# pinellolab/CRISPR-HAWK

Measured on AMD Instinct MI355X. Metric: candidate guides scored/sec, higher is better.
Workload: dtype u32

## Files before the change

### crispr-hawk_amd/csrc/hawk_api_cldict.hip

```cpp
#include <hip/hip_runtime.h>

#include <algorithm>
#include <cstdio>
#include <cstdlib>

#include "hawk_host.h"

static_assert(CL_MAX_ROWS == HAWK_ROW_MAX_HAP, "cl_build_sizes declines the rows the packed layout cannot hold");

enum ClBuildEvent { EV_BUILD_BEGIN = 8, EV_BUILD_END = 9 };

struct ClZero {
  char* base;
  const ClBuildSizes* z;
  template <class T> T* at(size_t off) const { return reinterpret_cast<T*>(base + off); }
  uint32_t* status() const { return at<uint32_t>(z->z_status); }
  uint32_t* counters() const { return at<uint32_t>(z->z_counters); }
  ClResults* results() const { return at<ClResults>(z->z_results); }
  uint32_t* cnt() const { return at<uint32_t>(z->z_cnt); }
  uint32_t* lcnt() const { return at<uint32_t>(z->z_lcnt); }
  uint32_t* claim() const { return at<uint32_t>(z->z_claim); }
  unsigned long long* vdesc() const { return at<unsigned long long>(z->z_vdesc); }
  uint32_t* span2() const { return at<uint32_t>(z->z_span2); }
  ClSlot* tab() const { return at<ClSlot>(z->z_tab); }
};

static int dict_reserve(hawk_xplan* x, const ClBuildSizes& sz, PoolScope& tmp, ClZero* zero, ClBuild* b) {
  ClusterDictionary& cl = x->cl;
  const uint32_t n = x->n_hap;
  zero->z = &sz;
  TEMPCHK(tmp, &zero->base, sz.z_end);
  ClChunks& ch = b->ch;
  TEMPCHK(tmp, &ch.ch_off, (size_t)(n + 1) * 4);
  TEMPCHK(tmp, &ch.ch_row, (size_t)sz.ch_bound * 4);
  TEMPCHK(tmp, &ch.inst_base, (size_t)(sz.ch_bound + 1) * 4);
  TEMPCHK(tmp, &ch.list_base, (size_t)(sz.ch_bound + 1) * 4);
  TEMPCHK(tmp, &b->list.list, (size_t)sz.inst_bound * sizeof(ClListed));
  TEMPCHK(tmp, &b->list.state, (size_t)sz.inst_bound * 4);
  for (DevBuf* buf : {&cl.inst_uid, &cl.inst_o, &cl.inst_row, &cl.inst_pa, &cl.inst_rb})
    if (int rc = buf->reserve((size_t)sz.inst_bound * 4)) return rc;
  ch.ch_bound = sz.ch_bound; ch.cnt = zero->cnt(); ch.lcnt = zero->lcnt();
  b->list.bound = sz.inst_bound;
  ClPlan& p = b->plan;
  p.heads = x->heads.p; p.hv_off = x->off.as<uint64_t>(); p.hap_len = x->hlen.as<uint32_t>();
  p.ss = x->m_ss.as<int32_t>(); p.se = x->m_se.as<int32_t>(); p.is_ref = x->m_is_ref.as<uint8_t>();
  p.seg_off = x->m_seg_off.as<uint32_t>(); p.seg_rel = x->m_seg_rel.as<uint32_t>();
  p.n_rows = n; p.n_var = x->n_var;
  b->var.desc = zero->vdesc(); b->var.claim = zero->claim();
  ClInst& ci = b->inst;
  ci.o = cl.inst_o.as<int32_t>(); ci.row = cl.inst_row.as<uint32_t>(); ci.pa = cl.inst_pa.as<int32_t>(); ci.rb = cl.inst_rb.as<int32_t>();
  ci.uid = cl.inst_uid.as<uint32_t>();
  b->tally.counters = zero->counters(); b->tally.results = zero->results(); b->tally.status = zero->status();
  return HAWK_OK;
}

static void dict_cut(hipStream_t st, const ClBuild& b) {
  const ClChunks& ch = b.ch;
  hawk_launch_cl_chunks(st, b);
  hawk_launch_cl_count(st, b);
  if (hawk_cl_head_chunks(ch.ch_bound))
    hawk_launch_scan2_u32(st, ch.cnt, ch.lcnt, ch.ch_bound, ch.inst_base, ch.list_base, b.var.desc, b.var.claim, b.plan.n_var);
  else
    hawk_launch_scan2_u32(st, ch.cnt, ch.lcnt, ch.ch_bound, ch.inst_base, ch.list_base);
}

static int dict_attempt(hawk_xplan* x, const ClBuild& b, const ClTable& t, uint32_t* span2, ClResults* res) {
  ClusterDictionary& cl = x->cl;
  hawk_ctx* ctx = x->ctx;
  hipStream_t st = ctx->stream;
  for (DevBuf* buf : {&cl.u_rec, &cl.u_n, &cl.u_row, &cl.u_o, &cl.u_seg})
    if (int rc = buf->reserve((size_t)t.u_cap * 4)) return rc;
  ClUniq cu;
  cu.rec = cl.u_rec.as<uint32_t>(); cu.n = cl.u_n.as<uint32_t>(); cu.row = cl.u_row.as<uint32_t>(); cu.o = cl.u_o.as<int32_t>();
  cu.seg = cl.u_seg.as<uint32_t>(); cu.span2 = span2;
  hawk_launch_cl_fill(st, b);
// ... 23 lines not shown
int xplan_build_dict(hawk_xplan* x) {
  ClusterDictionary& cl = x->cl;
  if (cl.built) return HAWK_OK;
  cl.built = true; cl.usable = false; cl.status = 0; cl.n_inst = cl.n_uniq = cl.n_real = 0; cl.slots = 0; cl.build_ms = 0.f;
  hawk_ctx* ctx = x->ctx;
  hipStream_t st = ctx->stream;
  const ClBuildSizes sz = cl_build_sizes(x->ncar, x->n_hap, x->n_var, cl.last_uniq);
  if (sz.declined) { cl.status = CL_ST_DECLINED; return HAWK_OK; }
  PoolScope tmp;
  ClZero zero;
  ClBuild b = {};
  int rc;
  if ((rc = dict_reserve(x, sz, tmp, &zero, &b))) return rc;
  HIPCHK(hipEventRecord(ctx->ev[EV_BUILD_BEGIN], st));
  HIPCHK(hipMemsetAsync(zero.base, 0, sz.z_end, st));
  dict_cut(st, b);
  ClResults* const res = &static_cast<PinnedBlock*>(ctx->pinned)->dict;
  *res = ClResults{};
  ClTable t;
  t.tab = zero.tab(); t.mask = sz.tsmall - 1; t.max_probe = sz.max_probe; t.fail_bit = sz.fail_bit; t.u_cap = sz.u_bound;
  if ((rc = dict_attempt(x, b, t, zero.span2(), res))) return rc;
  if (res->status & CL_ST_FIRST_TABLE) {
    const uint32_t status = (uint32_t)res->status & ~(uint32_t)CL_ST_FIRST_TABLE;
    HIPCHK(hipMemcpyAsync(zero.status(), &status, 4, hipMemcpyHostToDevice, st));
    uint32_t* d_span2;
    t.mask = sz.tsize - 1; t.max_probe = 0xffffffffu; t.fail_bit = CL_ST_COLLISION; t.u_cap = sz.u_bound_repeat;
    TEMPCHK(tmp, &d_span2, (size_t)t.u_cap * 4);
    TEMPCHK(tmp, &t.tab, (size_t)sz.tsize * sizeof(ClSlot));
    HIPCHK(hipMemsetAsync(t.tab, 0, (size_t)sz.tsize * sizeof(ClSlot), st));
    HIPCHK(hipMemsetAsync(d_span2, 0, (size_t)t.u_cap * 4, st));
    HIPCHK(hipMemsetAsync(zero.counters(), 0, sz.z_cnt - sz.z_counters, st));
    if ((rc = dict_attempt(x, b, t, d_span2, res))) return rc;
  }
  if (res->instances == 0) { cl.status = CL_ST_DECLINED; return HAWK_OK; }
  if ((uint32_t)res->instances > sz.inst_bound) { snprintf(hawk_hip_err_buf(), 256, "hawk_xplan_view: instance count beyond its bound"); return HAWK_E_HIP; }
  (void)hipEventElapsedTime(&cl.build_ms, ctx->ev[EV_BUILD_BEGIN], ctx->ev[EV_BUILD_END]);
  dict_decide(cl, *res, x->n_var, t.u_cap);
  return HAWK_OK;
}

extern "C" {

int hawk_xplan_cluster_stats(const hawk_xplan* x, uint32_t* usable, uint32_t* n_instances, uint32_t* n_distinct, uint64_t* template_slots,
                             float* build_ms, uint32_t* status) {
  if (!x) return HAWK_E_INVALID;
  if (usable) *usable = x->cl.built && x->cl.usable ? 1u : 0u;
  if (n_instances) *n_instances = x->cl.n_inst;
  if (n_distinct) *n_distinct = x->cl.n_real;
  if (template_slots) *template_slots = x->cl.slots;
  if (build_ms) *build_ms = x->cl.build_ms;
  if (status) *status = x->cl.built ? x->cl.status : 0xffffffffu;
  return HAWK_OK;
}

// ... 9 lines not shown
```

### crispr-hawk_amd/csrc/hawk_cl.h

```cpp
#pragma once
#include <stddef.h>
#include <stdint.h>

#define CL_LINK 64
#define CL_NONE 0xffffffffu
#define CL_FAR (1 << 29)
#define CL_ROW_U 4
#define CL_CHUNK (256 * CL_ROW_U)
#define CL_MAX_ROWS (1u << 23)

enum ClStatus : uint32_t {
  CL_ST_CHAIN = 1,
  CL_ST_COLLISION = 2,
  CL_ST_DECLINED = 4,
  CL_ST_FIRST_TABLE = 8,
};

struct ClInst {
  int32_t* o;
  uint32_t* row;
  int32_t* pa;
  int32_t* rb;
  uint32_t* uid;
};
struct ClUniq {
  uint32_t* rec; uint32_t* n; uint32_t* row; int32_t* o; uint32_t* seg; uint32_t* span2;
};
struct __attribute__((aligned(32))) ClSlot { unsigned long long key; unsigned long long pad; uint32_t up1, ncls, refp, var; };
static_assert(sizeof(ClSlot) == 32, "table slot layout");
struct __attribute__((aligned(32))) ClListed {
  uint32_t inst, key_lo, key_hi, rec, ncls, refp; int32_t o_first; uint32_t var;
};
static_assert(sizeof(ClListed) == 32, "list entry layout");

struct ClResults {
  unsigned long long instances, table_clusters, variant_clusters, template_rows, status, pad[3];
};
static_assert(sizeof(ClResults) == 64, "result block layout");

struct ClPlan {
  const void* heads;
  const uint64_t* hv_off;
  const uint32_t* hap_len;
  const int32_t* ss;
  const int32_t* se;
  const uint8_t* is_ref;
  const uint32_t* seg_off;
  const uint32_t* seg_rel;
  uint32_t n_rows, n_var;
};
struct ClChunks {
  uint32_t* ch_off;
  uint32_t* ch_row;
  uint32_t ch_bound;
  uint32_t* cnt;
  uint32_t* lcnt;
  uint32_t* inst_base;
  uint32_t* list_base;
};
struct ClVariants {
  unsigned long long* desc;
  uint32_t* claim;
};
struct ClList {
  ClListed* list;
  uint32_t* state;
  uint32_t bound;
};
struct ClTally {
  uint32_t* counters;
  ClResults* results;
  uint32_t* status;
};
struct ClBuild { ClPlan plan; ClChunks ch; ClVariants var; ClInst inst; ClList list; ClTally tally; };
struct ClTable {
  ClSlot* tab;
  uint32_t mask;
  uint32_t max_probe;
  uint32_t fail_bit;
  uint32_t u_cap;
};

inline uint32_t hawk_cl_chunk_bound(uint64_t n_records, uint32_t n_rows) { return (uint32_t)(n_records / CL_CHUNK) + n_rows; }

struct ClBuildSizes {
  bool declined;
  uint32_t ch_bound, inst_bound;
  uint32_t bm_words;
  uint32_t tsize, tsmall;
  uint32_t max_probe, fail_bit;
  uint32_t u_bound, u_bound_repeat;
  size_t z_status, z_counters, z_results, z_cnt, z_lcnt, z_claim, z_vdesc, z_span2, z_tab, z_end;
};
inline ClBuildSizes cl_build_sizes(uint64_t ncar, uint32_t n_rows, uint32_t n_var, uint32_t last_uniq) {
  ClBuildSizes s = {};
// ... 26 lines not shown
```

### crispr-hawk_amd/csrc/hawk_cldict.hip

```cpp
#include <cstdlib>

#include "hawk_hx.h"

#define CL_MAXWALK 4096

__device__ __forceinline__ uint64_t cl_mix(uint64_t h, uint64_t v) {
  h = (h ^ v) * 0x9E3779B97F4A7C15ull;
  return h ^ (h >> 29);
}
struct __attribute__((aligned(16))) HxHead { int32_t o; uint32_t rs; uint32_t alt_len; uint32_t var; };
static_assert(sizeof(HxHead) == 16, "record head layout");
__global__ __launch_bounds__(256) void k_hx_heads(const HxVar* __restrict__ recs, const uint32_t* __restrict__ hv_idx, uint64_t n, uint4* __restrict__ heads) {
  const uint64_t j = (uint64_t)blockIdx.x * 256 + threadIdx.x;
  if (j >= n) return;
  const uint4 r = *reinterpret_cast<const uint4*>(recs + j);
  heads[j] = make_uint4(r.x, r.y, r.z, hv_idx[j]);
}
void hawk_launch_hx_heads(hipStream_t st, const void* recs, const uint32_t* hv_idx, uint64_t n, void* heads) {
  if (n) hipLaunchKernelGGL(k_hx_heads, dim3((unsigned)((n + 255) / 256)), dim3(256), 0, st, static_cast<const HxVar*>(recs), hv_idx, n,
                            static_cast<uint4*>(heads));
}
__device__ __forceinline__ bool cl_starts(const HxHead* __restrict__ recs, uint64_t j, uint64_t lo) {
  if (j == lo) return true;
  const int32_t prev_end = recs[j - 1].o + (int32_t)recs[j - 1].alt_len;
// ... 102 lines not shown
      const uint64_t j = b0 + u * 256 + threadIdx.x;
      if (!(j < hi && (j == lo || (int32_t)r0[u].x - ((int32_t)rp[u].x + (int32_t)rp[u].z) > CL_LINK))) return;
      const ClCut k = cl_cut(recs, lo, hi, j, r0[u], rp[u], nx1, nx2, lane, ss, se, hl, row);
      const uint32_t v = r0[u].w;
      const bool simple = k.n == 1 && k.cls == 1 && v < n_var;
      c += 1u + ((k.cls != 0 && !simple) ? 0x10000u : 0u);
      if (simple && b < n_head) var_desc[v] = (unsigned long long)(uint32_t)j | ((unsigned long long)row << 32);
    };
    static_assert(CL_ROW_U == 4, "one call per slice");
    one(0); one(1); one(2); one(3);
  }
  uint32_t tot;
  (void)block_excl_scan<256 / WAVE>(c, s_w, &tot);
  if (threadIdx.x == 0) { cnt[b] = (tot & 0xffffu) + (b + 1 == ch_off[row + 1] ? 1u : 0u); lcnt[b] = tot >> 16; }
}

#define CL_BM_WORDS 4096
__global__ __launch_bounds__(256) void k_cl_fill(const HxHead* __restrict__ recs, const uint64_t* __restrict__ hv_off,
                                                 const uint32_t* __restrict__ hap_len, const int32_t* __restrict__ ss_,
                                                 const int32_t* __restrict__ se_, const uint32_t* __restrict__ ch_off,
                                                 const uint32_t* __restrict__ ch_row, const uint32_t* __restrict__ inst_base,
                                                 const uint32_t* __restrict__ list_base, ClInst ci, unsigned long long* __restrict__ var_desc,
                                                 const uint32_t* __restrict__ claim_bits, uint32_t n_var, ClListed* __restrict__ cx_list, uint32_t* __restrict__ status,
                                                 uint32_t n_rows) {
  __shared__ uint32_t s_c[256 / WAVE][CL_ROW_U];
  __shared__ uint32_t s_l[256 / WAVE][CL_ROW_U];
  __shared__ uint32_t s_bm[CL_BM_WORDS];
  const uint32_t b = blockIdx.x;
  if (b >= ch_off[n_rows]) return;
  const uint32_t row = ch_row[b];
  const uint64_t lo = hv_off[row], hi = hv_off[row + 1];
  const uint64_t b0 = lo + (uint64_t)(b - ch_off[row]) * CL_CHUNK;
  const int32_t ss = ss_[row], se = se_[row], hl = (int32_t)hap_len[row];
  const uint32_t lane = threadIdx.x & (WAVE - 1), wv = threadIdx.x / WAVE;
  const uint32_t at = inst_base[b], lat = list_base[b];
  uint32_t round_tot = 0;
  if (hi > lo) {
    const uint64_t b1 = b0 + CL_CHUNK < hi ? b0 + CL_CHUNK : hi;
    const uint32_t v_lo = recs[b0].var, v_hi = recs[b1 - 1].var;
    const uint32_t w_lo = v_lo >> 5, n_w = v_hi >= v_lo && v_hi < n_var ? (v_hi >> 5) - w_lo + 1u : 0u;
    const bool bm_lds = n_w != 0u && n_w <= CL_BM_WORDS;
    if (bm_lds) for (uint32_t w = threadIdx.x; w < n_w; w += 256) s_bm[w] = claim_bits[w_lo + w];
    uint4 r0[CL_ROW_U], rp[CL_ROW_U];
    bool st[CL_ROW_U];
    unsigned long long bal[CL_ROW_U];
#pragma unroll
    for (int u = 0; u < CL_ROW_U; ++u) {
// ... 13 lines not shown
    uint32_t pre[CL_ROW_U];
#pragma unroll
    for (int u = 0; u < CL_ROW_U; ++u) {
      pre[u] = round_tot;
#pragma unroll
      for (int w = 0; w < 256 / WAVE; ++w) {
        const uint32_t x = s_c[w][u];
        if (w < (int)wv) pre[u] += x;
        round_tot += x;
      }
    }
    uint4 ea[CL_ROW_U], eb[CL_ROW_U];
    bool listed[CL_ROW_U];
    unsigned long long lbal[CL_ROW_U];
    auto cut = [&](const int u) __attribute__((always_inline)) {
      const uint4 nx1 = shfl_down4(r0[u], 1), nx2 = shfl_down4(r0[u], 2);
      listed[u] = false;
      ea[u] = make_uint4(0u, 0u, 0u, 0u); eb[u] = ea[u];
      if (st[u]) {
        const uint64_t j = b0 + u * 256 + threadIdx.x;
        const uint32_t i = at + pre[u] + (uint32_t)__popcll(bal[u] & ((1ull << lane) - 1ull));
        const ClCut k = cl_cut(recs, lo, hi, j, r0[u], rp[u], nx1, nx2, lane, ss, se, hl, row);
        if (k.too_long) atomicOr(status, 1u);
        ci.o[i] = k.o_first; ci.row[i] = row; ci.pa[i] = k.pa | (k.run_inside ? (int32_t)0x80000000 : 0); ci.rb[i] = k.rb;
        const uint32_t v = r0[u].w;
        const bool simple = k.n == 1 && k.cls == 1 && v < n_var;
        if (!k.cls) ci.uid[i] = CL_NONE;
        if (simple) {
          ci.uid[i] = v;
          const uint32_t bit = 1u << (v & 31u);
          if (!((bm_lds ? s_bm[(v >> 5) - w_lo] : claim_bits[v >> 5]) & bit))
            var_desc[v] = (unsigned long long)(uint32_t)j | ((unsigned long long)row << 32);
        }
        listed[u] = k.cls != 0 && !simple;
        ea[u] = make_uint4(i, (uint32_t)k.key, (uint32_t)(k.key >> 32), (uint32_t)j);
        eb[u] = make_uint4(k.n | (k.cls << 16), (uint32_t)(k.o_first + k.rb), (uint32_t)k.o_first, v);
      }
      lbal[u] = __ballot(listed[u]);
      if (lane == 0) s_l[wv][u] = (uint32_t)__popcll(lbal[u]);
    };
    static_assert(CL_ROW_U == 4, "one call per slice");
    cut(0); cut(1); cut(2); cut(3);
    __syncthreads();
    uint32_t lpre = lat;
#pragma unroll
    for (int u = 0; u < CL_ROW_U; ++u) {
      uint32_t mine = lpre;
#pragma unroll
      for (int w = 0; w < 256 / WAVE; ++w) {
        const uint32_t x = s_l[w][u];
        if (w < (int)wv) mine += x;
        lpre += x;
      }
      if (listed[u]) {
        uint4* dst = reinterpret_cast<uint4*>(cx_list + mine + (uint32_t)__popcll(lbal[u] & ((1ull << lane) - 1ull)));
        dst[0] = ea[u]; dst[1] = eb[u];
      }
    }
  }
  if (threadIdx.x == 0 && b + 1 == ch_off[row + 1]) {
    const uint32_t i = at + round_tot;
    int32_t pa = 0, rb = 0;
    if (hi > lo) { pa = recs[hi - 1].o + (int32_t)recs[hi - 1].alt_len; rb = (int32_t)recs[hi - 1].rs - pa; }
    ci.o[i] = CL_FAR; ci.row[i] = row; ci.pa[i] = pa; ci.rb[i] = rb; ci.uid[i] = CL_NONE;
  }
}

#define CL_UID_U 4
__global__ __launch_bounds__(256) void k_cl_enter(const ClListed* __restrict__ cx_list, const uint32_t* __restrict__ n_list_dev, uint32_t t_first,
                                                  uint32_t t_end, ClSlot* tab, uint32_t mask, uint32_t max_probe, uint32_t fail_bit,
                                                  uint32_t* __restrict__ inst_uid, const uint32_t* __restrict__ inst_row, uint32_t* __restrict__ cx_state,
                                                  ClUniq cu, uint32_t* n_table, uint32_t n_var, uint32_t u_cap, uint32_t* __restrict__ status) {
  __shared__ uint32_t s_n[256 / WAVE][CL_UID_U];
  __shared__ uint32_t s_base;
  const uint32_t n_list = *n_list_dev < t_end ? *n_list_dev : t_end;
  const uint32_t t0 = t_first + blockIdx.x * (256 * CL_UID_U) + threadIdx.x;
  if (t_first + blockIdx.x * (256 * CL_UID_U) >= n_list) return;
  const uint32_t lane = threadIdx.x & (WAVE - 1), wv = threadIdx.x / WAVE;
  uint4 ent[CL_UID_U], lk[CL_UID_U];
  uint32_t sl[CL_UID_U];
  bool on[CL_UID_U], won[CL_UID_U];
#pragma unroll
  for (int u = 0; u < CL_UID_U; ++u) {
    const uint32_t t = t0 + u * 256;
    on[u] = t < n_list;
    ent[u] = *reinterpret_cast<const uint4*>(cx_list + (on[u] ? t : t_first));
  }
#pragma unroll
  for (int u = 0; u < CL_UID_U; ++u) {
    const unsigned long long k = (unsigned long long)ent[u].y | ((unsigned long long)ent[u].z << 32);
    sl[u] = (uint32_t)(k >> 17) & mask;
    lk[u] = *reinterpret_cast<const uint4*>(tab + sl[u]);
  }
#pragma unroll
  for (int u = 0; u < CL_UID_U; ++u) {
    won[u] = false;
    if (!on[u]) continue;
    const unsigned long long k = (unsigned long long)ent[u].y | ((unsigned long long)ent[u].z << 32);
    uint4 e0 = lk[u];
    uint32_t s = sl[u];
    bool placed = false;
    for (uint32_t probe = 0; probe <= mask && probe < max_probe; ++probe) {
      if (probe) e0 = *reinterpret_cast<const uint4*>(tab + s);
      unsigned long long c = (unsigned long long)e0.x | ((unsigned long long)e0.y << 32);
      if (c == 0ull) {
        c = atomicCAS(&tab[s].key, 0ull, k);
        won[u] = c == 0ull;
      }
      if (c == 0ull || c == k) { placed = true; break; }
      s = (s + 1u) & mask;
    }
    sl[u] = s;
    const uint32_t t = t0 + u * 256;
    if (!placed) { won[u] = false; cx_state[t] = CL_NONE; inst_uid[ent[u].x] = CL_NONE; atomicOr(status, fail_bit); continue; }
    cx_state[t] = won[u] ? CL_NONE : (CL_PENDING | s);
  }
  unsigned long long wb[CL_UID_U];
#pragma unroll
  for (int u = 0; u < CL_UID_U; ++u) { wb[u] = __ballot(won[u]); if (lane == 0) s_n[wv][u] = (uint32_t)__popcll(wb[u]); }
  __syncthreads();
  uint32_t tot = 0, mine[CL_UID_U];
#pragma unroll
  for (int u = 0; u < CL_UID_U; ++u) {
    mine[u] = tot;
#pragma unroll
    for (int w = 0; w < 256 / WAVE; ++w) { const uint32_t x = s_n[w][u]; if (w < (int)wv) mine[u] += x; tot += x; }
  }
  if (!tot) return;
  if (threadIdx.x == 0) s_base = atomicAdd(n_table, tot);
  __syncthreads();
  const uint32_t base = n_var + s_base;
#pragma unroll
  for (int u = 0; u < CL_UID_U; ++u) {
    if (!won[u]) continue;
    const uint32_t un = base + mine[u] + (uint32_t)__popcll(wb[u] & ((1ull << lane) - 1ull));
    const uint32_t i = ent[u].x;
    if (un >= u_cap) { inst_uid[i] = CL_NONE; atomicOr(status, fail_bit); continue; }
    const uint4 e1 = reinterpret_cast<const uint4*>(cx_list + (t0 + u * 256))[1];
    *reinterpret_cast<uint4*>(&tab[sl[u]].up1) = make_uint4(un + 1u, e1.x, e1.y, e1.w);
    inst_uid[i] = un;
    cu.rec[un] = ent[u].w; cu.n[un] = e1.x & 0xffffu; cu.row[un] = inst_row[i]; cu.o[un] = (int32_t)e1.z;
  }
}

__global__ __launch_bounds__(256) void k_cl_describe(const uint32_t* __restrict__ n_table_dev, uint32_t n_var, uint32_t u_cap,
                                                     const unsigned long long* __restrict__ var_desc, ClUniq cu, const HxHead* __restrict__ recs,
                                                     const uint32_t* __restrict__ seg_off, const uint32_t* __restrict__ seg_rel,
                                                     uint32_t* __restrict__ n_variant_clusters, unsigned long long* __restrict__ slots_total) {
  const uint32_t u = blockIdx.x * 256 + threadIdx.x;
  uint32_t span_u = 0;
  const uint32_t nu = n_var + *n_table_dev < u_cap ? n_var + *n_table_dev : u_cap;
  bool variant_cluster = false;
  if (u < nu) {
    uint32_t n, r, row;
    int32_t o_first;
    if (u < n_var) {
      const unsigned long long d = var_desc[u];
      variant_cluster = d != 0ull;
      r = (uint32_t)d; row = (uint32_t)(d >> 32); n = variant_cluster ? 1u : 0u;
      o_first = variant_cluster ? recs[r].o : 0;
      cu.rec[u] = r; cu.n[u] = n; cu.row[u] = row; cu.o[u] = o_first;
    } else {
      n = cu.n[u]; r = cu.rec[u]; row = cu.row[u]; o_first = cu.o[u];
    }
// ... 4 lines not shown
      cu.span2[u] = span_u;
      const uint32_t rel = o_first > CL_LINK + HAWK_PAD ? (uint32_t)(o_first - CL_LINK - HAWK_PAD) : 0u;
      uint32_t lo = seg_off[row], hi = seg_off[row + 1];
      while (hi - lo > 1) {
        const uint32_t mid = (lo + hi) >> 1;
        if (seg_rel[mid] <= rel) lo = mid; else hi = mid;
      }
      cu.seg[u] = lo;
    }
  }
  __shared__ uint32_t s_red[256 / WAVE][2];
  const unsigned long long vb = __ballot(variant_cluster);
  const uint32_t ssum = wave_sum(span_u);
  if ((threadIdx.x & (WAVE - 1)) == 0) { s_red[threadIdx.x / WAVE][0] = (uint32_t)__popcll(vb); s_red[threadIdx.x / WAVE][1] = ssum; }
  __syncthreads();
  if (threadIdx.x == 0) {
    uint32_t a = 0, b = 0;
#pragma unroll
    for (int w = 0; w < 256 / WAVE; ++w) { a += s_red[w][0]; b += s_red[w][1]; }
    if (a) atomicAdd(n_variant_clusters, a);
    if (b) atomicAdd(slots_total, (unsigned long long)b);
  }
}
__global__ void k_cl_results(const uint32_t* __restrict__ n_inst, const uint32_t* __restrict__ counters, const unsigned long long* __restrict__ slots_total,
                             const uint32_t* __restrict__ status, unsigned long long* __restrict__ out) {
  out[0] = *n_inst; out[1] = counters[0]; out[2] = counters[1]; out[3] = *slots_total; out[4] = *status;
}
__global__ __launch_bounds__(256) void k_cl_uid(const ClListed* __restrict__ cx_list, const uint32_t* __restrict__ n_list_dev, uint32_t t_end,
                                                const uint32_t* __restrict__ cx_state, const ClSlot* __restrict__ tab, uint32_t* __restrict__ inst_uid,
                                                ClUniq cu, const HxHead* __restrict__ recs, uint32_t* __restrict__ status) {
  const uint32_t n_list = *n_list_dev < t_end ? *n_list_dev : t_end;
  if (blockIdx.x * (256 * CL_UID_U) >= n_list) return;
  const uint32_t t0 = blockIdx.x * (256 * CL_UID_U) + threadIdx.x;
  uint32_t v[CL_UID_U];
  bool pend[CL_UID_U];
  bool any = false;
#pragma unroll
  for (int u = 0; u < CL_UID_U; ++u) {
    const uint32_t t = t0 + u * 256;
    v[u] = t < n_list ? cx_state[t] : CL_NONE;
    pend[u] = v[u] != CL_NONE && (v[u] & CL_PENDING);
    any = any || pend[u];
  }
  if (!__any(any)) return;
  uint4 e1[CL_UID_U], la[CL_UID_U], lb[CL_UID_U];
#pragma unroll
  for (int u = 0; u < CL_UID_U; ++u) {
    e1[u] = reinterpret_cast<const uint4*>(tab + (pend[u] ? (v[u] & ~CL_PENDING) : 0u))[1];
    const uint4* l = reinterpret_cast<const uint4*>(cx_list + (pend[u] ? t0 + u * 256 : 0u));
    la[u] = l[0]; lb[u] = l[1];
  }
  uint32_t rrec[CL_UID_U];
#pragma unroll
  for (int u = 0; u < CL_UID_U; ++u) rrec[u] = (pend[u] && e1[u].x != 0u && (lb[u].x & 0xffffu) > 1u) ? cu.rec[e1[u].x - 1u] : 0u;
  bool bad = false;
#pragma unroll
  for (int u = 0; u < CL_UID_U; ++u) {
    if (!pend[u]) continue;
    const uint32_t i = la[u].x, ncls = lb[u].x;
    if (e1[u].x == 0u) { inst_uid[i] = CL_NONE; bad = true; continue; }
    inst_uid[i] = e1[u].x - 1u;
    bool b = ncls != e1[u].y || (ncls >> 16) != 1 || lb[u].y != e1[u].z || lb[u].w != e1[u].w;
    const uint32_t n = ncls & 0xffffu;
    if (!b && n > 1) {
      const HxHead* pa = recs + la[u].w;
      const HxHead* pb = recs + rrec[u];
      const int32_t oa = (int32_t)lb[u].z, ob = pb[0].o;
      for (uint32_t k = 1; k < n; ++k) {
        const uint4 xa = *reinterpret_cast<const uint4*>(pa + k), xb = *reinterpret_cast<const uint4*>(pb + k);
        b = b || xa.w != xb.w || xa.z != xb.z || xa.y != xb.y || (int32_t)xa.x - oa != (int32_t)xb.x - ob;
      }
    }
    bad = bad || b;
  }
  if (bad) atomicOr(status, 2u);
}

void hawk_launch_cl_chunks(hipStream_t st, const ClBuild& b) {
  hipLaunchKernelGGL(k_cl_chunks, dim3(1), dim3(1024), 0, st, b.plan.hv_off, b.plan.is_ref, b.plan.ss, b.plan.se, b.plan.n_rows, b.ch.ch_off, b.ch.ch_row);
}
#define CL_HEAD_CHUNKS 96
#define CL_HEAD_LISTED 16384
uint32_t hawk_cl_head_chunks(uint32_t ch_bound) { return ch_bound < 16 * CL_HEAD_CHUNKS ? 0u : CL_HEAD_CHUNKS; }
void hawk_launch_cl_count(hipStream_t st, const ClBuild& b) {
  const ClPlan& p = b.plan;
  if (b.ch.ch_bound)
    hipLaunchKernelGGL(k_cl_count, dim3(b.ch.ch_bound), dim3(256), 0, st, static_cast<const HxHead*>(p.heads), p.hv_off, p.hap_len, p.ss, p.se, b.ch.ch_off,
                       b.ch.ch_row, p.n_rows, p.n_var, b.ch.cnt, b.ch.lcnt, b.var.desc, hawk_cl_head_chunks(b.ch.ch_bound));
}
void hawk_launch_cl_fill(hipStream_t st, const ClBuild& b) {
  const ClPlan& p = b.plan;
#ifdef HAWK_TEST_HOOKS
  {
    const char* wk = getenv("HAWK_CLUSTER_WEAK_HASH");
    const uint32_t weak = wk && wk[0] == '1' ? 1u : 0u;
    (void)hipMemcpyToSymbol(HIP_SYMBOL(cl_weak_hash), &weak, sizeof(weak));
  }
#endif
  if (b.ch.ch_bound)
    hipLaunchKernelGGL(k_cl_fill, dim3(b.ch.ch_bound), dim3(256), 0, st, static_cast<const HxHead*>(p.heads), p.hv_off, p.hap_len, p.ss, p.se, b.ch.ch_off,
                       b.ch.ch_row, b.ch.inst_base, b.ch.list_base, b.inst, b.var.desc, b.var.claim, p.n_var, b.list.list, b.tally.status, p.n_rows);
}
void hawk_launch_cl_finish(hipStream_t st, const ClBuild& b, const ClTable& t, const ClUniq& cu) {
  const ClPlan& p = b.plan;
  const HxHead* recs = static_cast<const HxHead*>(p.heads);
  const uint32_t* n_inst_dev = b.ch.inst_base + b.ch.ch_bound;
  const uint32_t* n_list_dev = b.ch.list_base + b.ch.ch_bound;
  uint32_t* counters = b.tally.counters;
  uint32_t* status = b.tally.status;
  const uint32_t list_bound = b.list.bound;
  const uint32_t per = 256 * CL_UID_U;
  const uint32_t head = list_bound < 16 * CL_HEAD_LISTED ? 0u : CL_HEAD_LISTED;
  if (head)
    hipLaunchKernelGGL(k_cl_enter, dim3((head + per - 1) / per), dim3(256), 0, st, b.list.list, n_list_dev, 0u, head, t.tab, t.mask, t.max_probe,
                       t.fail_bit, b.inst.uid, b.inst.row, b.list.state, cu, counters, p.n_var, t.u_cap, status);
  if (list_bound > head)
    hipLaunchKernelGGL(k_cl_enter, dim3((list_bound - head + per - 1) / per), dim3(256), 0, st, b.list.list, n_list_dev, head, list_bound, t.tab,
                       t.mask, t.max_probe, t.fail_bit, b.inst.uid, b.inst.row, b.list.state, cu, counters, p.n_var, t.u_cap, status);
  hipLaunchKernelGGL(k_cl_describe, dim3((t.u_cap + 255) / 256), dim3(256), 0, st, counters, p.n_var, t.u_cap, b.var.desc, cu, recs, p.seg_off, p.seg_rel,
                     counters + 1, reinterpret_cast<unsigned long long*>(counters + 4));
  if (list_bound)
    hipLaunchKernelGGL(k_cl_uid, dim3((list_bound + per - 1) / per), dim3(256), 0, st, b.list.list, n_list_dev, list_bound, b.list.state, t.tab, b.inst.uid, cu,
                       recs, status);
  hipLaunchKernelGGL(k_cl_results, dim3(1), dim3(1), 0, st, n_inst_dev, counters, reinterpret_cast<const unsigned long long*>(counters + 4), status,
                     &b.tally.results->instances);
}
```

### crispr-hawk_amd/csrc/hawk_csearch.hip

```cpp
#include "hawk_vc.h"

#define CS_G 8

size_t hawk_cs_row_bytes() { return sizeof(CsRow); }

__device__ __forceinline__ VcRanges cs_ranges(const HapSetDev& hs, const ScanParams& p, uint32_t h) {
  VcRanges rg;
  const int ss = hs.scan_start[h], se = hs.scan_stop[h], haplen = (int)hs.hap_len[h];
  const int poF = p.right ? 0 : p.guidelen, poR = p.right ? p.guidelen : 0;
  const int qmin = HAWK_PAD, qmax = haplen - p.L - HAWK_PAD + 1;
  rg.slo[0] = ss - poF; rg.shi[0] = se - poF; rg.slo[1] = ss - poR; rg.shi[1] = se - poR;
  rg.lo[0] = rg.slo[0] > qmin ? rg.slo[0] : qmin; rg.hi[0] = rg.shi[0] < qmax ? rg.shi[0] : qmax;
  rg.lo[1] = rg.slo[1] > qmin ? rg.slo[1] : qmin; rg.hi[1] = rg.shi[1] < qmax ? rg.shi[1] : qmax;
  return rg;
}
__device__ __forceinline__ uint32_t group_incl_scan(uint32_t v, uint32_t gl) {
#pragma unroll
  for (int d = 1; d < CS_G; d <<= 1) {
    const uint32_t t = (uint32_t)__shfl_up((int)v, d, CS_G);
    if (gl >= (uint32_t)d) v += t;
  }
  return v;
}

// ... 234 lines not shown
}
__device__ __forceinline__ void cs_inst_store(uint4* q, const uint4& v) { *q = v; }
__device__ __forceinline__ uint4 cs_inst_load(const uint4* q) {
  typedef uint32_t u32x4 __attribute__((ext_vector_type(4)));
  const u32x4 v = __builtin_nontemporal_load(reinterpret_cast<const u32x4*>(q));
  return make_uint4(v.x, v.y, v.z, v.w);
}
#define CS_CNT_U 4
__global__ __launch_bounds__(256) void k_cs_count(HapSetDev hs, VcArgs va, ClDict cd, ScanParams p, const uint4* __restrict__ res,
                                                  const unsigned long long* __restrict__ t_count, uint64_t t_cap,
                                                  uint32_t* __restrict__ group_counts, uint4* __restrict__ inst, unsigned long long* __restrict__ shards) {
  __shared__ uint32_t s_red[256 / WAVE][2];
  const uint32_t i0 = blockIdx.x * (256 * CS_CNT_U) + threadIdx.x;
  const uint32_t lane = threadIdx.x & (WAVE - 1);
  const bool ovf = *t_count > t_cap;
  uint32_t uid[CS_CNT_U], below[CS_CNT_U], row[CS_CNT_U];
  int32_t paf[CS_CNT_U], o[CS_CNT_U];
  bool in[CS_CNT_U];
#pragma unroll
  for (int u = 0; u < CS_CNT_U; ++u) {
    const uint32_t i = i0 + u * 256;
    in[u] = i < cd.n_inst;
    const uint32_t ic = in[u] ? i : 0u;
    uid[u] = __builtin_nontemporal_load(cd.inst_uid + ic); paf[u] = __builtin_nontemporal_load(cd.inst_pa + ic);
    row[u] = __builtin_nontemporal_load(cd.inst_row + ic); o[u] = __builtin_nontemporal_load(cd.inst_o + ic);
    below[u] = CL_NONE;
    if (lane == 0 && in[u] && i > 0) below[u] = cd.inst_uid[i - 1];
  }
  uint4 r[CS_CNT_U], r2[CS_CNT_U];
  uint32_t behind0[CS_CNT_U];
#pragma unroll
  for (int u = 0; u < CS_CNT_U; ++u) {
    const bool has = in[u] && uid[u] != CL_NONE;
    r[u] = make_uint4(0u, 0u, 0u, 0u); r2[u] = r[u]; behind0[u] = 0u;
    if (cd.n_uniq) {
      const uint32_t us = has ? uid[u] : 0u;
      r[u] = res[2 * us]; r2[u] = res[2 * us + 1];
      if (lane == 0 && below[u] != CL_NONE) behind0[u] = res[2 * below[u] + 1].z;
    }
    if (!has) { r[u] = make_uint4(0u, 0u, 0u, 0u); r2[u] = r[u]; }
  }
  uint32_t cand = 0, hits = 0;
#pragma unroll
  for (int u = 0; u < CS_CNT_U; ++u) {
    const uint32_t i = i0 + u * 256;
    uint32_t behind = (uint32_t)__shfl_up((int)r2[u].z, 1);
    if (lane == 0) behind = behind0[u];
    uint32_t rows_i = 0;
    if (in[u]) {
      if (paf[u] < 0) {
// ... 222 lines not shown
  m.win[3 * m.cap + i] = (uint64_t)d.x | ((uint64_t)d.y << 32);
  m.win[4 * m.cap + i] = (uint64_t)d.z | ((uint64_t)d.w << 32);
}
__global__ __launch_bounds__(256) void k_cc_gidm(const uint32_t* __restrict__ perm, const uint64_t* __restrict__ goff, uint64_t nm, uint64_t G,
                                                 uint32_t* __restrict__ gidm) {
  const uint64_t j = (uint64_t)blockIdx.x * 256 + threadIdx.x;
  if (j >= nm) return;
  uint64_t lo = 0, hi = G;
  while (hi - lo > 1) {
    const uint64_t mid = (lo + hi) >> 1;
    if (goff[mid] <= j) lo = mid; else hi = mid;
  }
  gidm[perm[j]] = (uint32_t)lo;
}
__global__ __launch_bounds__(256) void k_cs_gid(ClDict cd, const uint4* __restrict__ res, const uint64_t* __restrict__ moff,
                                                const uint64_t* __restrict__ offsets, uint64_t r0, uint64_t n, const uint32_t* __restrict__ gidm,
                                                uint32_t* __restrict__ gid, uint32_t* __restrict__ vals) {
  __shared__ uint32_t s_ex[4][WAVE + 1];
  __shared__ uint32_t s_tb[4][WAVE];
  const uint32_t wv = threadIdx.x / WAVE, lane = threadIdx.x & (WAVE - 1);
  const uint32_t i = blockIdx.x * 256 + threadIdx.x;
  uint32_t cnt = 0, tb = 0;
  if (i < cd.n_inst) {
    const uint32_t u = cd.inst_uid[i];
    if (u != CL_NONE) { const uint4 r = res[2 * u]; cnt = r.x + r.y; tb = (uint32_t)moff[u]; }
  }
  const uint32_t inc = wave_incl_scan(cnt);
  const uint32_t Wt = (uint32_t)__builtin_amdgcn_readlane((int)inc, WAVE - 1);
  const uint32_t i0 = blockIdx.x * 256 + wv * WAVE;
  const uint64_t o0 = i0 < cd.n_inst ? offsets[i0 / WAVE] : 0;
  s_ex[wv][lane] = inc - cnt;
  s_tb[wv][lane] = tb;
  __syncthreads();
  if (o0 + Wt > n) return;
  for (uint32_t t = lane; t < Wt; t += WAVE) {
    uint32_t l = 0;
#pragma unroll
    for (uint32_t step = WAVE / 2; step; step >>= 1) l += (s_ex[wv][l + step] <= t) ? step : 0u;
    const uint64_t o = o0 + t;
    gid[o] = gidm[r0 + s_tb[wv][l] + (t - s_ex[wv][l])];
    vals[o] = (uint32_t)o;
  }
}
__global__ __launch_bounds__(256) void k_cc_refgid(uint64_t r0, const uint32_t* __restrict__ gidm, uint32_t* __restrict__ gid, uint32_t* __restrict__ vals) {
  const uint64_t i = (uint64_t)blockIdx.x * 256 + threadIdx.x;
  if (i < r0) { gid[i] = gidm[i]; vals[i] = (uint32_t)i; }
}
// ... 19 lines not shown
```

### crispr-hawk_amd/csrc/hawk_device.h

```cpp
#pragma once
#include <hip/hip_runtime.h>
#include <stdint.h>

#include "hawk_cl.h"

#define HAWK_PLANES 5
#define HAWK_PAD 10
#define HAWK_BLOCK 256
#define HAWK_WPT 4

struct HapSetDev {
  uint32_t n_hap;
  uint32_t S;
  const uint32_t* plane[HAWK_PLANES];
  const uint32_t* hap_len;
  const uint8_t* is_ref;
  const int32_t* scan_start;
  const int32_t* scan_stop;
  const uint32_t* seg_off;
  const uint32_t* seg_rel;
  const int64_t* seg_gen;
  int32_t ref_index;
};

// ... 73 lines not shown

struct RefInfo {
  int32_t index;
  int32_t lo[2], hi[2];
  int64_t startp;
  const uint32_t* bits[2];
  uint32_t n_bits;
};
struct VcArgs {
  const uint32_t* ref[4];
  uint32_t ref_S;
  const void* recs_;
  const uint8_t* alt_codes;
  const uint64_t* hv_off;
  const void* tiles_;
  const uint4* hp;
};
void hawk_launch_vsearch(hipStream_t st, int pass, const HapSetDev& hs, const VcArgs& va, const ScanParams& p, const struct GuideParams& gp,
                         const struct RefInfo& ri, const TileMeta* tmeta, uint32_t* counts, uint32_t* counts0, unsigned long long* shards,
                         const uint64_t* offsets, struct GuideCols out, int* status, uint32_t tile0, uint32_t n_tiles);
void hawk_launch_ref_hits(hipStream_t st, const HapSetDev& hs, const ScanParams& p, int32_t ref_index, void* hp);
struct ClDict {
  uint32_t n_inst, n_uniq;
  const uint32_t* inst_uid;
  const int32_t* inst_o;
  const uint32_t* inst_row;
  const int32_t* inst_pa;
  const int32_t* inst_rb;
  const uint32_t* u_rec;
  const uint32_t* u_n;
  const uint32_t* u_row;
  const int32_t* u_o;
  const uint32_t* u_seg;
};
size_t hawk_cs_row_bytes();
void hawk_launch_scan2_u32(hipStream_t st, const uint32_t* cnt_a, const uint32_t* cnt_b, uint32_t n, uint32_t* off_a, uint32_t* off_b,
                           const void* desc = nullptr, uint32_t* desc_bits = nullptr, uint32_t n_desc = 0);
void hawk_launch_hx_heads(hipStream_t st, const void* recs, const uint32_t* hv_idx, uint64_t n, void* heads);
void hawk_launch_cl_chunks(hipStream_t st, const ClBuild& b);
uint32_t hawk_cl_head_chunks(uint32_t ch_bound);
void hawk_launch_cl_count(hipStream_t st, const ClBuild& b);
void hawk_launch_cl_fill(hipStream_t st, const ClBuild& b);
void hawk_launch_cl_finish(hipStream_t st, const ClBuild& b, const ClTable& t, const ClUniq& cu);
void hawk_launch_cs_templates(hipStream_t st, const HapSetDev& hs, const VcArgs& va, const ClDict& cd, const ScanParams& p, const struct GuideParams& gp,
                              const struct RefInfo& ri, void* res , uint32_t* tbase, void* trows,
                              unsigned long long* t_count, uint64_t t_cap, int* status);
void hawk_launch_cs_count(hipStream_t st, const HapSetDev& hs, const VcArgs& va, const ClDict& cd, const ScanParams& p, const void* res,
                          const unsigned long long* t_count, uint64_t t_cap, uint32_t* group_counts, void* inst ,
                          unsigned long long* shards);
void hawk_launch_cs_emit_rows(hipStream_t st, uint32_t n_inst, const void* inst, const void* trows, const uint64_t* offsets,
// ... 321 lines not shown
```

### crispr-hawk_amd/csrc/hawk_host.h

```cpp
#pragma once
#include <hip/hip_runtime.h>

#include <cstddef>
#include <cstdio>
#include <initializer_list>
#include <memory>
#include <utility>
#include <vector>

#include "../../include/hawk.h"
#include "hawk_device.h"

#define HAWK_MAX_DEVICES 16
char* hawk_hip_err_buf();

#define HIPCHK(expr)                                                                         \
  do {                                                                                       \
    hipError_t e_ = (expr);                                                                  \
    if (e_ != hipSuccess) {                                                                  \
      snprintf(hawk_hip_err_buf(), 256, "%s: %s (%s:%d)", #expr, hipGetErrorString(e_), __FILE__, __LINE__); \
      return HAWK_E_HIP;                                                                     \
    }                                                                                        \
  } while (0)

// ... 153 lines not shown
  DevBuf otsum;
  DevBuf big;
  DevBuf refbits;
  bool refbits_valid = false;
  uint64_t refbits_key[6] = {0, 0, 0, 0, 0, 0};
  const struct hawk_xplan* vplan = nullptr;
  DevBuf vcnt0;
  DevBuf refhp;
  uint64_t cs_tcap = 0;
  DevBuf cs_res, cs_tbase, cs_trows, cs_inst;
  DevBuf colsA[8];
  DevBuf rowsA;
  uint64_t rows_cap = 0;
};

struct ClusterDictionary {
  bool built = false, usable = false;
  uint32_t n_inst = 0, n_uniq = 0;
  uint32_t n_real = 0;
  uint32_t last_uniq = 0;
  uint64_t slots = 0;
  uint32_t status = 0;
  float build_ms = 0.f;
  DevBuf inst_uid, inst_o, inst_row, inst_pa, inst_rb, u_rec, u_n, u_row, u_o, u_seg;
  void release() {
    for (DevBuf* b : {&inst_uid, &inst_o, &inst_row, &inst_pa, &inst_rb, &u_rec, &u_n, &u_row, &u_o, &u_seg}) b->release();
  }
  ClDict view() const {
    ClDict cd;
    cd.n_inst = n_inst; cd.n_uniq = n_uniq;
    cd.inst_uid = inst_uid.as<uint32_t>(); cd.inst_o = inst_o.as<int32_t>(); cd.inst_row = inst_row.as<uint32_t>();
    cd.inst_pa = inst_pa.as<int32_t>(); cd.inst_rb = inst_rb.as<int32_t>();
    cd.u_rec = u_rec.as<uint32_t>(); cd.u_n = u_n.as<uint32_t>(); cd.u_row = u_row.as<uint32_t>(); cd.u_o = u_o.as<int32_t>();
    cd.u_seg = u_seg.as<uint32_t>();
    return cd;
  }
};

struct hawk_xplan {
  hawk_ctx* ctx;
  uint32_t n_var, n_hap, ref_len;
  uint64_t ncar;
  std::vector<uint32_t> hap_len;
  uint32_t* ref_plane[4];
  uint32_t ref_S;
  DevBuf ref5[HAWK_PLANES];
  DevBuf recs, tiles, codes, off, hlen, hash;
  DevBuf heads;
  bool has_meta;
  std::vector<int32_t> scan_start, scan_stop;
  DevBuf m_is_ref, m_ss, m_se, m_seg_off, m_seg_rel, m_seg_gen, m_tile;
  uint32_t nseg, bph, S;
  int32_t ref_index;
  int64_t ref_startp, min_gen, max_gen;
  bool has_partner = false;
// ... 72 lines not shown
```

Baseline: 652.7 billion.

## Pack per-instance cluster fields into 16-byte records and drop results kernel

Replaces the four separate per-instance arrays (uid, pa, row, o) with one aligned 16-byte record, so fill writes it with a single vector store and the search kernel reads it with one 128-bit load instead of four scattered loads. Counters and status now live directly inside the results struct, which removes the single-thread k_cl_results kernel launch. The fill kernel now writes the instance count itself, and rb is written only when it is needed. In exchange, the uid updates in the enter and uid kernels become strided partial writes into the records.

```diff
diff --git a/crispr-hawk_amd/csrc/hawk_api_cldict.hip b/crispr-hawk_amd/csrc/hawk_api_cldict.hip
--- a/crispr-hawk_amd/csrc/hawk_api_cldict.hip
+++ b/crispr-hawk_amd/csrc/hawk_api_cldict.hip
@@ -14,8 +14,6 @@
   char* base;
   const ClBuildSizes* z;
   template <class T> T* at(size_t off) const { return reinterpret_cast<T*>(base + off); }
-  uint32_t* status() const { return at<uint32_t>(z->z_status); }
-  uint32_t* counters() const { return at<uint32_t>(z->z_counters); }
   ClResults* results() const { return at<ClResults>(z->z_results); }
   uint32_t* cnt() const { return at<uint32_t>(z->z_cnt); }
   uint32_t* lcnt() const { return at<uint32_t>(z->z_lcnt); }
@@ -37,8 +35,8 @@
   TEMPCHK(tmp, &ch.list_base, (size_t)(sz.ch_bound + 1) * 4);
   TEMPCHK(tmp, &b->list.list, (size_t)sz.inst_bound * sizeof(ClListed));
   TEMPCHK(tmp, &b->list.state, (size_t)sz.inst_bound * 4);
-  for (DevBuf* buf : {&cl.inst_uid, &cl.inst_o, &cl.inst_row, &cl.inst_pa, &cl.inst_rb})
-    if (int rc = buf->reserve((size_t)sz.inst_bound * 4)) return rc;
+  if (int rc = cl.inst.reserve((size_t)sz.inst_bound * sizeof(ClInstRec))) return rc;
+  if (int rc = cl.inst_rb.reserve((size_t)sz.inst_bound * 4)) return rc;
   ch.ch_bound = sz.ch_bound; ch.cnt = zero->cnt(); ch.lcnt = zero->lcnt();
   b->list.bound = sz.inst_bound;
   ClPlan& p = b->plan;
@@ -47,10 +45,8 @@
   p.seg_off = x->m_seg_off.as<uint32_t>(); p.seg_rel = x->m_seg_rel.as<uint32_t>();
   p.n_rows = n; p.n_var = x->n_var;
   b->var.desc = zero->vdesc(); b->var.claim = zero->claim();
-  ClInst& ci = b->inst;
-  ci.o = cl.inst_o.as<int32_t>(); ci.row = cl.inst_row.as<uint32_t>(); ci.pa = cl.inst_pa.as<int32_t>(); ci.rb = cl.inst_rb.as<int32_t>();
-  ci.uid = cl.inst_uid.as<uint32_t>();
-  b->tally.counters = zero->counters(); b->tally.results = zero->results(); b->tally.status = zero->status();
+  b->inst.rec = cl.inst.as<ClInstRec>(); b->inst.rb = cl.inst_rb.as<int32_t>();
+  b->tally.results = zero->results();
   return HAWK_OK;
 }
 
@@ -120,14 +116,14 @@
   if ((rc = dict_attempt(x, b, t, zero.span2(), res))) return rc;
   if (res->status & CL_ST_FIRST_TABLE) {
     const uint32_t status = (uint32_t)res->status & ~(uint32_t)CL_ST_FIRST_TABLE;
-    HIPCHK(hipMemcpyAsync(zero.status(), &status, 4, hipMemcpyHostToDevice, st));
     uint32_t* d_span2;
     t.mask = sz.tsize - 1; t.max_probe = 0xffffffffu; t.fail_bit = CL_ST_COLLISION; t.u_cap = sz.u_bound_repeat;
     TEMPCHK(tmp, &d_span2, (size_t)t.u_cap * 4);
     TEMPCHK(tmp, &t.tab, (size_t)sz.tsize * sizeof(ClSlot));
     HIPCHK(hipMemsetAsync(t.tab, 0, (size_t)sz.tsize * sizeof(ClSlot), st));
     HIPCHK(hipMemsetAsync(d_span2, 0, (size_t)t.u_cap * 4, st));
-    HIPCHK(hipMemsetAsync(zero.counters(), 0, sz.z_cnt - sz.z_counters, st));
+    HIPCHK(hipMemsetAsync(zero.results(), 0, sizeof(ClResults), st));
+    HIPCHK(hipMemcpyAsync(b.tally.status(), &status, 4, hipMemcpyHostToDevice, st));
     if ((rc = dict_attempt(x, b, t, d_span2, res))) return rc;
   }
   if (res->instances == 0) { cl.status = CL_ST_DECLINED; return HAWK_OK; }
diff --git a/crispr-hawk_amd/csrc/hawk_cl.h b/crispr-hawk_amd/csrc/hawk_cl.h
--- a/crispr-hawk_amd/csrc/hawk_cl.h
+++ b/crispr-hawk_amd/csrc/hawk_cl.h
@@ -16,12 +16,16 @@
   CL_ST_FIRST_TABLE = 8,
 };
 
+struct __attribute__((aligned(16))) ClInstRec {
+  uint32_t uid;
+  int32_t pa;
+  uint32_t row;
+  int32_t o;
+};
+static_assert(sizeof(ClInstRec) == 16 && alignof(ClInstRec) == 16, "instance record layout");
 struct ClInst {
-  int32_t* o;
-  uint32_t* row;
-  int32_t* pa;
+  ClInstRec* rec;
   int32_t* rb;
-  uint32_t* uid;
 };
 struct ClUniq {
   uint32_t* rec; uint32_t* n; uint32_t* row; int32_t* o; uint32_t* seg; uint32_t* span2;
@@ -68,9 +72,10 @@
   uint32_t bound;
 };
 struct ClTally {
-  uint32_t* counters;
   ClResults* results;
-  uint32_t* status;
+  uint32_t* table_clusters() const { return reinterpret_cast<uint32_t*>(&results->table_clusters); }
+  uint32_t* variant_clusters() const { return reinterpret_cast<uint32_t*>(&results->variant_clusters); }
+  uint32_t* status() const { return reinterpret_cast<uint32_t*>(&results->status); }
 };
 struct ClBuild { ClPlan plan; ClChunks ch; ClVariants var; ClInst inst; ClList list; ClTally tally; };
 struct ClTable {
diff --git a/crispr-hawk_amd/csrc/hawk_cldict.hip b/crispr-hawk_amd/csrc/hawk_cldict.hip
--- a/crispr-hawk_amd/csrc/hawk_cldict.hip
+++ b/crispr-hawk_amd/csrc/hawk_cldict.hip
@@ -148,7 +148,7 @@
                                                  const uint32_t* __restrict__ ch_row, const uint32_t* __restrict__ inst_base,
                                                  const uint32_t* __restrict__ list_base, ClInst ci, unsigned long long* __restrict__ var_desc,
                                                  const uint32_t* __restrict__ claim_bits, uint32_t n_var, ClListed* __restrict__ cx_list, uint32_t* __restrict__ status,
-                                                 uint32_t n_rows) {
+                                                 unsigned long long* __restrict__ n_instances, uint32_t n_rows) {
   __shared__ uint32_t s_c[256 / WAVE][CL_ROW_U];
   __shared__ uint32_t s_l[256 / WAVE][CL_ROW_U];
   __shared__ uint32_t s_bm[CL_BM_WORDS];
@@ -208,12 +208,11 @@
         const uint32_t i = at + pre[u] + (uint32_t)__popcll(bal[u] & ((1ull << lane) - 1ull));
         const ClCut k = cl_cut(recs, lo, hi, j, r0[u], rp[u], nx1, nx2, lane, ss, se, hl, row);
         if (k.too_long) atomicOr(status, 1u);
-        ci.o[i] = k.o_first; ci.row[i] = row; ci.pa[i] = k.pa | (k.run_inside ? (int32_t)0x80000000 : 0); ci.rb[i] = k.rb;
         const uint32_t v = r0[u].w;
         const bool simple = k.n == 1 && k.cls == 1 && v < n_var;
-        if (!k.cls) ci.uid[i] = CL_NONE;
+        *reinterpret_cast<uint4*>(ci.rec + i) = make_uint4(simple ? v : CL_NONE, (uint32_t)k.pa | (k.run_inside ? 0x80000000u : 0u), row, (uint32_t)k.o_first);
+        if (!k.run_inside) ci.rb[i] = k.rb;
         if (simple) {
-          ci.uid[i] = v;
           const uint32_t bit = 1u << (v & 31u);
           if (!((bm_lds ? s_bm[(v >> 5) - w_lo] : claim_bits[v >> 5]) & bit))
             var_desc[v] = (unsigned long long)(uint32_t)j | ((unsigned long long)row << 32);
@@ -248,14 +247,16 @@
     const uint32_t i = at + round_tot;
     int32_t pa = 0, rb = 0;
     if (hi > lo) { pa = recs[hi - 1].o + (int32_t)recs[hi - 1].alt_len; rb = (int32_t)recs[hi - 1].rs - pa; }
-    ci.o[i] = CL_FAR; ci.row[i] = row; ci.pa[i] = pa; ci.rb[i] = rb; ci.uid[i] = CL_NONE;
+    *reinterpret_cast<uint4*>(ci.rec + i) = make_uint4(CL_NONE, (uint32_t)pa, row, (uint32_t)CL_FAR);
+    ci.rb[i] = rb;
+    if (b + 1 == ch_off[n_rows]) *n_instances = (unsigned long long)i + 1u;
   }
 }
 
 #define CL_UID_U 4
 __global__ __launch_bounds__(256) void k_cl_enter(const ClListed* __restrict__ cx_list, const uint32_t* __restrict__ n_list_dev, uint32_t t_first,
                                                   uint32_t t_end, ClSlot* tab, uint32_t mask, uint32_t max_probe, uint32_t fail_bit,
-                                                  uint32_t* __restrict__ inst_uid, const uint32_t* __restrict__ inst_row, uint32_t* __restrict__ cx_state,
+                                                  ClInstRec* __restrict__ inst, uint32_t* __restrict__ cx_state,
                                                   ClUniq cu, uint32_t* n_table, uint32_t n_var, uint32_t u_cap, uint32_t* __restrict__ status) {
   __shared__ uint32_t s_n[256 / WAVE][CL_UID_U];
   __shared__ uint32_t s_base;
@@ -298,7 +299,7 @@
     }
     sl[u] = s;
     const uint32_t t = t0 + u * 256;
-    if (!placed) { won[u] = false; cx_state[t] = CL_NONE; inst_uid[ent[u].x] = CL_NONE; atomicOr(status, fail_bit); continue; }
+    if (!placed) { won[u] = false; cx_state[t] = CL_NONE; inst[ent[u].x].uid = CL_NONE; atomicOr(status, fail_bit); continue; }
     cx_state[t] = won[u] ? CL_NONE : (CL_PENDING | s);
   }
   unsigned long long wb[CL_UID_U];
@@ -321,11 +322,11 @@
     if (!won[u]) continue;
     const uint32_t un = base + mine[u] + (uint32_t)__popcll(wb[u] & ((1ull << lane) - 1ull));
     const uint32_t i = ent[u].x;
-    if (un >= u_cap) { inst_uid[i] = CL_NONE; atomicOr(status, fail_bit); continue; }
+    if (un >= u_cap) { inst[i].uid = CL_NONE; atomicOr(status, fail_bit); continue; }
     const uint4 e1 = reinterpret_cast<const uint4*>(cx_list + (t0 + u * 256))[1];
     *reinterpret_cast<uint4*>(&tab[sl[u]].up1) = make_uint4(un + 1u, e1.x, e1.y, e1.w);
-    inst_uid[i] = un;
-    cu.rec[un] = ent[u].w; cu.n[un] = e1.x & 0xffffu; cu.row[un] = inst_row[i]; cu.o[un] = (int32_t)e1.z;
+    cu.rec[un] = ent[u].w; cu.n[un] = e1.x & 0xffffu; cu.row[un] = inst[i].row; cu.o[un] = (int32_t)e1.z;
+    inst[i].uid = un;
   }
 }
 
@@ -376,12 +377,8 @@
     if (b) atomicAdd(slots_total, (unsigned long long)b);
   }
 }
-__global__ void k_cl_results(const uint32_t* __restrict__ n_inst, const uint32_t* __restrict__ counters, const unsigned long long* __restrict__ slots_total,
-                             const uint32_t* __restrict__ status, unsigned long long* __restrict__ out) {
-  out[0] = *n_inst; out[1] = counters[0]; out[2] = counters[1]; out[3] = *slots_total; out[4] = *status;
-}
 __global__ __launch_bounds__(256) void k_cl_uid(const ClListed* __restrict__ cx_list, const uint32_t* __restrict__ n_list_dev, uint32_t t_end,
-                                                const uint32_t* __restrict__ cx_state, const ClSlot* __restrict__ tab, uint32_t* __restrict__ inst_uid,
+                                                const uint32_t* __restrict__ cx_state, const ClSlot* __restrict__ tab, ClInstRec* __restrict__ inst,
                                                 ClUniq cu, const HxHead* __restrict__ recs, uint32_t* __restrict__ status) {
   const uint32_t n_list = *n_list_dev < t_end ? *n_list_dev : t_end;
   if (blockIdx.x * (256 * CL_UID_U) >= n_list) return;
@@ -412,8 +409,8 @@
   for (int u = 0; u < CL_UID_U; ++u) {
     if (!pend[u]) continue;
     const uint32_t i = la[u].x, ncls = lb[u].x;
-    if (e1[u].x == 0u) { inst_uid[i] = CL_NONE; bad = true; continue; }
-    inst_uid[i] = e1[u].x - 1u;
+    if (e1[u].x == 0u) { inst[i].uid = CL_NONE; bad = true; continue; }
+    inst[i].uid = e1[u].x - 1u;
     bool b = ncls != e1[u].y || (ncls >> 16) != 1 || lb[u].y != e1[u].z || lb[u].w != e1[u].w;
     const uint32_t n = ncls & 0xffffu;
     if (!b && n > 1) {
@@ -453,29 +450,27 @@
 #endif
   if (b.ch.ch_bound)
     hipLaunchKernelGGL(k_cl_fill, dim3(b.ch.ch_bound), dim3(256), 0, st, static_cast<const HxHead*>(p.heads), p.hv_off, p.hap_len, p.ss, p.se, b.ch.ch_off,
-                       b.ch.ch_row, b.ch.inst_base, b.ch.list_base, b.inst, b.var.desc, b.var.claim, p.n_var, b.list.list, b.tally.status, p.n_rows);
+                       b.ch.ch_row, b.ch.inst_base, b.ch.list_base, b.inst, b.var.desc, b.var.claim, p.n_var, b.list.list, b.tally.status(),
+                       &b.tally.results->instances, p.n_rows);
 }
 void hawk_launch_cl_finish(hipStream_t st, const ClBuild& b, const ClTable& t, const ClUniq& cu) {
   const ClPlan& p = b.plan;
   const HxHead* recs = static_cast<const HxHead*>(p.heads);
-  const uint32_t* n_inst_dev = b.ch.inst_base + b.ch.ch_bound;
   const uint32_t* n_list_dev = b.ch.list_base + b.ch.ch_bound;
-  uint32_t* counters = b.tally.counters;
-  uint32_t* status = b.tally.status;
+  uint32_t* n_table = b.tally.table_clusters();
+  uint32_t* status = b.tally.status();
   const uint32_t list_bound = b.list.bound;
   const uint32_t per = 256 * CL_UID_U;
   const uint32_t head = list_bound < 16 * CL_HEAD_LISTED ? 0u : CL_HEAD_LISTED;
   if (head)
     hipLaunchKernelGGL(k_cl_enter, dim3((head + per - 1) / per), dim3(256), 0, st, b.list.list, n_list_dev, 0u, head, t.tab, t.mask, t.max_probe,
-                       t.fail_bit, b.inst.uid, b.inst.row, b.list.state, cu, counters, p.n_var, t.u_cap, status);
+                       t.fail_bit, b.inst.rec, b.list.state, cu, n_table, p.n_var, t.u_cap, status);
   if (list_bound > head)
     hipLaunchKernelGGL(k_cl_enter, dim3((list_bound - head + per - 1) / per), dim3(256), 0, st, b.list.list, n_list_dev, head, list_bound, t.tab,
-                       t.mask, t.max_probe, t.fail_bit, b.inst.uid, b.inst.row, b.list.state, cu, counters, p.n_var, t.u_cap, status);
-  hipLaunchKernelGGL(k_cl_describe, dim3((t.u_cap + 255) / 256), dim3(256), 0, st, counters, p.n_var, t.u_cap, b.var.desc, cu, recs, p.seg_off, p.seg_rel,
-                     counters + 1, reinterpret_cast<unsigned long long*>(counters + 4));
+                       t.mask, t.max_probe, t.fail_bit, b.inst.rec, b.list.state, cu, n_table, p.n_var, t.u_cap, status);
+  hipLaunchKernelGGL(k_cl_describe, dim3((t.u_cap + 255) / 256), dim3(256), 0, st, n_table, p.n_var, t.u_cap, b.var.desc, cu, recs, p.seg_off, p.seg_rel,
+                     b.tally.variant_clusters(), &b.tally.results->template_rows);
   if (list_bound)
-    hipLaunchKernelGGL(k_cl_uid, dim3((list_bound + per - 1) / per), dim3(256), 0, st, b.list.list, n_list_dev, list_bound, b.list.state, t.tab, b.inst.uid, cu,
+    hipLaunchKernelGGL(k_cl_uid, dim3((list_bound + per - 1) / per), dim3(256), 0, st, b.list.list, n_list_dev, list_bound, b.list.state, t.tab, b.inst.rec, cu,
                        recs, status);
-  hipLaunchKernelGGL(k_cl_results, dim3(1), dim3(1), 0, st, n_inst_dev, counters, reinterpret_cast<const unsigned long long*>(counters + 4), status,
-                     &b.tally.results->instances);
-}
+}
diff --git a/crispr-hawk_amd/csrc/hawk_csearch.hip b/crispr-hawk_amd/csrc/hawk_csearch.hip
--- a/crispr-hawk_amd/csrc/hawk_csearch.hip
+++ b/crispr-hawk_amd/csrc/hawk_csearch.hip
@@ -280,10 +280,10 @@
     const uint32_t i = i0 + u * 256;
     in[u] = i < cd.n_inst;
     const uint32_t ic = in[u] ? i : 0u;
-    uid[u] = __builtin_nontemporal_load(cd.inst_uid + ic); paf[u] = __builtin_nontemporal_load(cd.inst_pa + ic);
-    row[u] = __builtin_nontemporal_load(cd.inst_row + ic); o[u] = __builtin_nontemporal_load(cd.inst_o + ic);
+    const uint4 rec = cs_inst_load(reinterpret_cast<const uint4*>(cd.inst + ic));
+    uid[u] = rec.x; paf[u] = (int32_t)rec.y; row[u] = rec.z; o[u] = (int32_t)rec.w;
     below[u] = CL_NONE;
-    if (lane == 0 && in[u] && i > 0) below[u] = cd.inst_uid[i - 1];
+    if (lane == 0 && in[u] && i > 0) below[u] = cd.inst[i - 1].uid;
   }
   uint4 r[CS_CNT_U], r2[CS_CNT_U];
   uint32_t behind0[CS_CNT_U];
@@ -552,7 +552,7 @@
   const uint32_t i = blockIdx.x * 256 + threadIdx.x;
   uint32_t cnt = 0, tb = 0;
   if (i < cd.n_inst) {
-    const uint32_t u = cd.inst_uid[i];
+    const uint32_t u = cd.inst[i].uid;
     if (u != CL_NONE) { const uint4 r = res[2 * u]; cnt = r.x + r.y; tb = (uint32_t)moff[u]; }
   }
   const uint32_t inc = wave_incl_scan(cnt);
diff --git a/crispr-hawk_amd/csrc/hawk_device.h b/crispr-hawk_amd/csrc/hawk_device.h
--- a/crispr-hawk_amd/csrc/hawk_device.h
+++ b/crispr-hawk_amd/csrc/hawk_device.h
@@ -119,10 +119,7 @@
 void hawk_launch_ref_hits(hipStream_t st, const HapSetDev& hs, const ScanParams& p, int32_t ref_index, void* hp);
 struct ClDict {
   uint32_t n_inst, n_uniq;
-  const uint32_t* inst_uid;
-  const int32_t* inst_o;
-  const uint32_t* inst_row;
-  const int32_t* inst_pa;
+  const ClInstRec* inst;
   const int32_t* inst_rb;
   const uint32_t* u_rec;
   const uint32_t* u_n;
diff --git a/crispr-hawk_amd/csrc/hawk_host.h b/crispr-hawk_amd/csrc/hawk_host.h
--- a/crispr-hawk_amd/csrc/hawk_host.h
+++ b/crispr-hawk_amd/csrc/hawk_host.h
@@ -199,15 +199,14 @@
   uint64_t slots = 0;
   uint32_t status = 0;
   float build_ms = 0.f;
-  DevBuf inst_uid, inst_o, inst_row, inst_pa, inst_rb, u_rec, u_n, u_row, u_o, u_seg;
+  DevBuf inst, inst_rb, u_rec, u_n, u_row, u_o, u_seg;
   void release() {
-    for (DevBuf* b : {&inst_uid, &inst_o, &inst_row, &inst_pa, &inst_rb, &u_rec, &u_n, &u_row, &u_o, &u_seg}) b->release();
+    for (DevBuf* b : {&inst, &inst_rb, &u_rec, &u_n, &u_row, &u_o, &u_seg}) b->release();
   }
   ClDict view() const {
     ClDict cd;
     cd.n_inst = n_inst; cd.n_uniq = n_uniq;
-    cd.inst_uid = inst_uid.as<uint32_t>(); cd.inst_o = inst_o.as<int32_t>(); cd.inst_row = inst_row.as<uint32_t>();
-    cd.inst_pa = inst_pa.as<int32_t>(); cd.inst_rb = inst_rb.as<int32_t>();
+    cd.inst = inst.as<ClInstRec>(); cd.inst_rb = inst_rb.as<int32_t>();
     cd.u_rec = u_rec.as<uint32_t>(); cd.u_n = u_n.as<uint32_t>(); cd.u_row = u_row.as<uint32_t>(); cd.u_o = u_o.as<int32_t>();
     cd.u_seg = u_seg.as<uint32_t>();
     return cd;
```

Result: no change. 649.0 billion (-0.6%).
